# slp-rl/aero

Hardware: AMD Instinct MI355X
Metric: real-time-factor (audio-sec/wall-sec), Aero.forward STFT+U-Net+iSTFT, 4->16kHz nfft=512 hop=64 batch=64 per GPU (higher is better)
Workload: dtype f16; 1 GPU; batch=64 synthetic 2s white-noise clips per GPU, 4->16 kHz, aero_4-16_512_64 (nfft=512 hop=64), random-init weights seed 2036, inference, inputs resident in HBM; global_batch=64, clip_samples=8000, frames=501, parallelism=clips sharded over 1 GPU(s), no data-path collective, precision=fp16 operands/storage, fp32 accumulate; STFT/iSTFT/statistics fp32

## Files before the change

aero_amd/_lib.py:

```python
import ctypes as C
import os

_HERE = os.path.dirname(os.path.abspath(__file__))
DEFAULT_LIB = os.path.join(_HERE, 'libaero_hip.so')

ACT_NONE, ACT_RELU, ACT_GELU, ACT_GLU, ACT_SNAKE = 0, 1, 2, 3, 4

i32, i64, vp, fp, dp = C.c_int32, C.c_int64, C.c_void_p, C.c_void_p, C.c_void_p


class ConvDesc(C.Structure):
    _fields_ = [('src0', vp), ('s0_b', i64), ('s0_f', i64), ('s0_t', i64), ('C0', i32),
                ('src1', vp), ('s1_b', i64), ('s1_f', i64), ('s1_t', i64), ('C1', i32),
                ('weight', vp), ('bias', fp),
                ('dst', vp), ('d_b', i64), ('d_f', i64), ('d_t', i64),
                ('dst_f32', i32), ('dst_f_off', i32), ('dst_F', i32),
                ('B', i32), ('Fin', i32), ('Fout', i32), ('T', i32), ('M', i32),
                ('transposed', i32), ('fstride', i32),
                ('ntaps', i32), ('df', i32 * 9), ('dt', i32 * 9),
                ('act', i32),
                ('res', vp), ('r_b', i64), ('r_f', i64), ('r_t', i64),
                ('post_add', fp), ('batch_scale', fp), ('batch_shift', fp),
                ('stats', dp), ('stat_count', C.c_double),
                ('stat_mode', i32), ('stat_G', i32), ('stat_per_row', i32), ('stat_eps', C.c_float),
# ... 98 lines not shown
    _fields_ = [('xn', vp), ('u', vp), ('g', vp), ('rs', fp), ('a_re', fp), ('a_im', fp), ('bias_f', fp),
                ('wc', vp), ('bias_c', fp), ('dst', vp),
                ('B', i32), ('F', i32), ('T', i32), ('C', i32), ('M', i32), ('Fo', i32), ('ktaps', i32), ('stride', i32),
                ('pad', i32), ('act', i32)]


class SeanetConvDesc(C.Structure):
    _fields_ = [('x', vp), ('wimg', vp), ('bias', fp), ('add', vp), ('y', vp),
                ('B', i32), ('Tin', i32), ('Cin', i32), ('Tq', i32), ('M', i32), ('K', i32), ('stride', i32), ('dil', i32), ('pad', i32),
                ('reflect', i32), ('ksteps', i32), ('R', i32), ('P', i32), ('Tout', i32), ('Cout', i32), ('act', i32), ('in_slope', C.c_float)]


class SeanetResDesc(C.Structure):
    _fields_ = [('x', vp), ('w1', vp), ('w2s', vp), ('b1', fp), ('b2s', fp), ('add', vp), ('y', vp),
                ('B', i32), ('T', i32), ('C', i32), ('d', i32), ('ks1', i32), ('ks2', i32), ('slope', C.c_float)]


DCONV_MAX_DEPTH = 4


class DconvLayer(C.Structure):
    _fields_ = [('w1', vp), ('w2', vp), ('consts', fp), ('snake_a', fp),
                ('dilation', i32), ('norm1', i32), ('norm2', i32), ('reserved', i32)]


class DconvDesc(C.Structure):
    _fields_ = [('x', vp), ('y', vp), ('R', i32), ('T', i32), ('C', i32), ('hidden', i32), ('depth', i32), ('act', i32),
                ('F', i32), ('eps', C.c_float), ('layer', DconvLayer * DCONV_MAX_DEPTH)]


class DconvRewriteDesc(C.Structure):
    _fields_ = [('dconv', DconvDesc), ('rw_w', vp), ('rw_bias', fp), ('post_add', fp),
                ('dst', vp), ('d_b', i64), ('d_f', i64), ('d_t', i64)]


_PROTOS = {
    'aero_version': (C.c_char_p, []),
    'aero_last_error': (C.c_char_p, []),
    'aero_last_kernel_name': (C.c_char_p, []),
    'aero_stft_fwd': (i32, [fp, i32, i32, i32, i32, i32, fp, i32, fp, i32, dp, i32, vp]),
    'aero_stft_dft_table_bytes': (i64, [i32]),
    'aero_stft_dft_table': (i32, [fp, i32, i32, vp, vp]),
    'aero_stft_dft_fwd': (i32, [fp, i32, i32, i32, i32, i32, i32, vp, fp, i32, dp, i32, vp]),
    'aero_stft_dft_norm_fwd': (i32, [fp, i32, i32, i32, i32, i32, i32, vp, i32, dp, i32, vp, fp, vp]),
    'aero_spec_normalize': (i32, [fp, i32, i64, dp, vp, fp, vp]),
    'aero_istft_fwd': (i32, [fp, i32, i32, i32, i32, i32, fp, fp, fp, i32, vp]),
    'aero_istft_pitch': (i32, [i32, i32, i32, C.POINTER(i32), C.POINTER(i32)]),
    'aero_istft_pitched_fwd': (i32, [fp, i32, i32, i32, i32, i32, i32, i32, fp, fp, fp, i32, vp]),
    'aero_conv_fwd': (i32, [C.POINTER(ConvDesc), vp]),
    'aero_split_finish': (i32, [fp, i32, fp, i32, vp, i64, i32, vp]),
    'aero_adam_step': (i32, [fp, fp, fp, fp, i64, C.c_float, C.c_float, C.c_float, C.c_float, i32, C.c_float, vp]),
    'aero_adam_step_dev': (i32, [fp, fp, fp, fp, i64, C.c_float, C.c_float, C.c_float, C.c_float, fp, C.c_float, vp]),
    'aero_conv_wgrad': (i32, [C.POINTER(WgradDesc), vp]),
    'aero_conv_wgrad_chunks': (i32, [i32, i32, i32, i32, i32]),
    'aero_norm_bwd_reduce': (i32, [C.POINTER(NormBwdDesc), vp]),
    'aero_norm_bwd_apply': (i32, [C.POINTER(NormBwdDesc), vp]),
    'aero_istft_bwd_prep': (i32, [fp, fp, fp, i32, i32, i32, i32, i32, vp]),
    'aero_istft_bwd_pack': (i32, [fp, fp, i32, i32, i32, i32, i32, vp]),
    'aero_conv_tile_m': (i32, [i32]),
    'aero_conv_ring_bm': (i32, [i32, i32]),
    'aero_convtr_tail_finish': (i32, [fp, fp, fp, fp, fp, fp, i32, i32, i32, i32, i32, vp]),
    'aero_convtr_tail_finish_pitched': (i32, [fp, fp, fp, fp, fp, fp, i32, i32, i32, i32, i32, i32, i32, vp]),
    'aero_conv_kernel_name': (i32, [C.POINTER(ConvDesc), C.c_char_p, i32]),
    'aero_norm_stats': (i32, [C.POINTER(NormDesc), vp]),
    'aero_norm_apply': (i32, [C.POINTER(NormDesc), vp]),
    'aero_gram_stats': (i32, [C.POINTER(GramDesc), vp]),
    'aero_lstm_fwd': (i32, [C.POINTER(LstmDesc), vp]),
    'aero_lstm_geometry': (i32, [i32, C.POINTER(i32), C.POINTER(i32)]),
    'aero_lstm_geometry_in': (i32, [i32, i32, C.POINTER(i32)]),
    'aero_localstate_fwd': (i32, [C.POINTER(AttnDesc), vp]),
    'aero_freqfc_fwd': (i32, [C.POINTER(FreqFcDesc), vp]),
    'aero_ftb_first_fwd': (i32, [C.POINTER(FtbFirstDesc), vp]),
    'aero_enc0_fwd': (i32, [C.POINTER(Enc0Desc), vp]),
    'aero_dconv_row_fwd': (i32, [C.POINTER(DconvDesc), vp]),
    'aero_dconv_row_fits': (i32, [i32, i32, i32, i32]),
    'aero_dconv_row_rewrite_fwd': (i32, [C.POINTER(DconvRewriteDesc), vp]),
    'aero_dconv_row_rewrite_fits': (i32, [i32, i32, i32, i32]),
    'aero_lstm_bwd': (i32, [C.POINTER(LstmBwdDesc), vp]),
    'aero_lstm_bwd_k4p': (i32, [i32]),
    'aero_localstate_bwd': (i32, [C.POINTER(AttnBwdDesc), vp]),
    'aero_freqfc_wgrad': (i32, [vp, vp, vp, fp, fp, i32, i32, i32, i32, i32, vp]),
    'aero_ftb_gate_bwd': (i32, [vp, vp, vp, vp, vp, vp, i32, i32, i32, i32, vp]),
    'aero_sum_bt': (i32, [vp, fp, i32, i32, i32, i32, C.c_float, vp]),
    'aero_frames_op': (i32, [vp, vp, i32, i32, i32, i32, i32, i32, i32, vp]),
    'aero_stft_loss_sums': (i32, [fp, fp, i64, C.c_float, dp, i32, dp, vp]),
    'aero_stft_loss_bwd': (i32, [fp, fp, i64, C.c_float, dp, C.c_float, C.c_float, fp, fp, vp]),
    'aero_irfft_frames': (i32, [fp, i32, i32, i32, i32, fp, fp, vp]),
    'aero_stft_adj_fold': (i32, [fp, fp, i32, i32, i32, i32, i32, i32, vp]),
    'aero_add_f16': (i32, [vp, vp, vp, i64, C.c_float, vp]),
    'aero_scale_cast': (i32, [fp, i32, i64, fp, vp, C.c_float, vp, fp, vp]),
    'aero_scale_f32': (i32, [fp, i64, fp, vp]),
    'aero_gather_pack': (i32, [vp, vp, i32, vp, vp, i64, i32, vp]),
    'aero_debug_probe': (i32, [vp, i32, i32, i32, vp, vp]),
    'aero_bn_running_update': (i32, [dp, i32, C.c_double, C.c_float, fp, fp, vp, vp]),
    'aero_gconv1d_mfma_ok': (i32, [i32, i32, i32, i32, i32, i32, i32]),
    'aero_weightnorm_fwd': (i32, [fp, fp, fp, i32, i32, vp]),
    'aero_weightnorm_bwd': (i32, [fp, i64, i64, i64, fp, fp, fp, fp, fp, fp, fp, fp, i32, i32, i32, i32, vp]),
    'aero_gconv1d_wgrad_slabs': (i32, [i32, i32, i32, i32, i32, i32, i32, i32, i32]),
    'aero_rescale_f16': (i32, [vp, fp, vp, fp, i64, vp, C.c_float, vp, fp, vp]),
    'aero_gconv1d_fwd': (i32, [C.POINTER(GconvDesc), vp]),
    'aero_pw_fwd': (i32, [C.POINTER(PwDesc), vp]),
    'aero_comm_unique_id': (i32, [vp]),
    'aero_comm_init': (i32, [i32, i32, vp, C.POINTER(vp)]),
    'aero_allreduce_f32': (i32, [vp, fp, i64, vp]),
    'aero_allgather': (i32, [vp, vp, vp, i64, vp]),
    'aero_comm_destroy': (i32, [vp]),
    'aero_stream_create': (i32, [i32, C.POINTER(C.c_uint32), i32, C.POINTER(vp)]),
    'aero_stream_destroy': (i32, [vp]),
    'aero_pw_rows': (i32, [i32, i32]),
    'aero_pw_ksteps': (i32, [i32]),
# ... 78 lines not shown
```

aero_amd/csrc/aero_hip.hip:

```cpp
#include "aero_common.h"
#ifdef AERO_PART
#define AERO_IN(p) (AERO_PART == (p))
#else
#define AERO_IN(p) 1
#endif
#if AERO_IN(0)
#include "k_attn.h"
#include "k_lstm.h"
#include "k_norm.h"
#include "k_gram.h"
#include "k_optim.h"
#endif
#if AERO_IN(1)
#include "k_stft.h"
#include "k_train.h"
#endif
#if AERO_IN(2)
#include "k_conv.h"
#endif
#if AERO_IN(6)
#include "k_conv_ring.h"
#endif
#if AERO_IN(7)
#include "k_pw.h"
// ... 414 lines not shown
int aero_split_finish(const float* acc, int32_t nsplit, const float* bias, int32_t act, void* dst, int64_t npos, int32_t M, void* stream) {
    const char* err = "";
    int rc = aero_split_finish_launch(acc, nsplit, bias, act, dst, npos, M, (hipStream_t)stream, &err);
    return aero_finish(rc, err);
}

#endif

#if AERO_IN(3)

int aero_freqfc_fwd(const aero_freqfc_desc* d, void* stream) {
    const char* err = "";
    int rc = aero_freqfc_launch(d, (hipStream_t)stream, &err);
    return aero_finish(rc, err);
}

int aero_dconv_row_fwd(const aero_dconv_desc* d, void* stream) {
    const char* err = "";
    int rc = aero_dconv_launch(d, nullptr, (hipStream_t)stream, &err);
    return aero_finish(rc, err);
}

int aero_dconv_row_fits(int T, int C, int hidden, int max_dilation) { return aero_dconv_row_fits_impl(T, C, hidden, max_dilation); }

int aero_dconv_row_rewrite_fwd(const aero_dconv_rewrite_desc* d, void* stream) {
    const char* err = "";
    if (!d) return aero_fail(AERO_ERR_ARG, "dconv rewrite: null descriptor");
    int rc = aero_dconv_launch(&d->dconv, d, (hipStream_t)stream, &err);
    return aero_finish(rc, err);
}

int aero_dconv_row_rewrite_fits(int T, int C, int hidden, int max_dilation) { return aero_dconv_row_fits_impl(T, C, hidden, max_dilation, true); }

int aero_enc0_fwd(const aero_enc0_desc* d, void* stream) {
    const char* err = "";
    int rc = aero_enc0_launch(d, (hipStream_t)stream, &err);
    return aero_finish(rc, err);
}

int aero_ftb_first_fwd(const aero_ftb_first_desc* d, void* stream) {
    const char* err = "";
    int rc = aero_ftb_first_launch(d, (hipStream_t)stream, &err);
    return aero_finish(rc, err);
}

#endif

#if AERO_IN(4)

int aero_conv_wgrad(const aero_wgrad_desc* d, void* stream) {
    const char* err = "";
    int rc = aero_conv_wgrad_launch(d, (hipStream_t)stream, &err);
    return aero_finish(rc, err);
}

int aero_conv_wgrad_chunks(int32_t M, int32_t C, int32_t ntaps, int32_t nrows, int32_t T) {
    if (M < 1 || C < 1 || ntaps < 1 || nrows < 1 || T < 1) return 1;
    bool big;
    int nchunk, SC;
    aero_wgrad_plan(M, C, ntaps, nrows, T, &big, &nchunk, &SC);
    return nchunk;
}

int aero_norm_bwd_reduce(const aero_norm_bwd_desc* d, void* stream) {
    const char* err = "";
    int rc = aero_norm_bwd_launch(d, 0, (hipStream_t)stream, &err);
// ... 338 lines not shown
```

aero_amd/csrc/k_dconv.h:

```cpp
#pragma once
#include "aero_common.h"

struct AeroDconvK {
    aero_dconv_desc d;
    int HP;
    int logp;
    int T16;
    int PADR;
    const void* rw_w;
    const float* rw_b;
    const float* rw_add;
    void* out; int64_t o_b, o_f, o_t;
};

static inline int aero_dconv_logp(int C) {
    int s = (2 * C) & 255, g = 256;
    if (s) g = s & -s;
    int P = 256 / g, l = 0;
    while ((1 << l) < P) ++l;
    return l;
}

static inline size_t aero_dconv_lds_bytes(int T, int C, int hidden, int maxdil) {
    if (T < 1 || C < 8 || C % 8 || hidden < 4 || hidden % 4 || hidden > 32 || maxdil < 1 || maxdil > 64) return 0;
// ... 324 lines not shown
    p.rw_b = rw ? rw->rw_bias : nullptr;
    p.rw_add = rw ? rw->post_add : nullptr;
    p.out = rw ? rw->dst : nullptr;
    p.o_b = rw ? rw->d_b : 0; p.o_f = rw ? rw->d_f : 0; p.o_t = rw ? rw->d_t : 0;
    const size_t lds = rw ? aero_dconv_rw_lds_bytes(d->T, d->C, d->hidden, maxdil) : aero_dconv_lds_bytes(d->T, d->C, d->hidden, maxdil);
    const int nw = aero_dconv_nw(lds, d->T), nf2 = d->C / 8;
    dim3 grid((unsigned)d->R), block((unsigned)nw * 64);
#define AERO_DCONV_GO2(NF2_, RW_)                                                                                      \
    do {                                                                                                               \
        constexpr int MF16 = NF2_ >= 12 ? 2 : 4;      \
        if (nw == 16 && (d->T + 15) / 16 > 16 * MF16) { *err = "dconv: row too long"; return AERO_ERR_UNSUPPORTED; }    \
        if (p.HP == 16 && nw == 8) AERO_LAUNCH_DYN((aero_dconv_row_kernel<1, NF2_, 8, 4, RW_>), grid, block, lds, stream, p);  \
        else if (p.HP == 16) AERO_LAUNCH_DYN((aero_dconv_row_kernel<1, NF2_, 16, MF16, RW_>), grid, block, lds, stream, p);       \
        else if (nw == 8) AERO_LAUNCH_DYN((aero_dconv_row_kernel<2, NF2_, 8, 4, RW_>), grid, block, lds, stream, p);           \
        else AERO_LAUNCH_DYN((aero_dconv_row_kernel<2, NF2_, 16, MF16, RW_>), grid, block, lds, stream, p);                       \
    } while (0)
#define AERO_DCONV_GO(NF2_)                                                                                            \
    do {                                                                                                               \
        if (rw) AERO_DCONV_GO2(NF2_, true);                                                                            \
        else AERO_DCONV_GO2(NF2_, false);                                                                              \
    } while (0)
    switch (nf2) {
        case 2: AERO_DCONV_GO(2); break;
        case 4: AERO_DCONV_GO(4); break;
        case 6: AERO_DCONV_GO(6); break;
        case 8: AERO_DCONV_GO(8); break;
        case 12: AERO_DCONV_GO(12); break;
        default: AERO_DCONV_GO(16); break;
    }
#undef AERO_DCONV_GO
#undef AERO_DCONV_GO2
    return AERO_OK;
}
```

aero_amd/engine.py:

```python
import ctypes as C
import math
import os

import torch

from . import _lib, pack
from ._lib import ACT_GELU, ACT_GLU, ACT_NONE, ACT_RELU, ACT_SNAKE


def _ptr(t):
    return None if t is None else t.data_ptr()


def _strides4(t):
    assert t.dim() == 4 and (t.shape[3] == 1 or t.stride(3) == 1), (t.shape, t.stride())
    return t.stride(0), t.stride(1), t.stride(2)


_SIDE_STREAMS = {}


def side_streams(device, n):
    dev = torch.device(device)
    if dev.type == 'cuda' and dev.index is None:
# ... 285 lines not shown
            ar[0].zero_()
        ar[1] = ar[2] = 0
        self._cur = ar

    _bwd = None

    def zeros32(self, n, device, dtype=torch.float32):
        ar = self._bwd
        if ar is not None and ar[0].device == torch.device(device):
            m = (n + 3) // 4 * 4
            ar[2] += m
            if ar[1] + m <= ar[0].numel():
                out = ar[0][ar[1]:ar[1] + n]
                ar[1] += m
                return out if dtype == torch.float32 else out.view(dtype)
        return torch.zeros(n, dtype=dtype, device=device)

    def new_stats(self, B, F, G, per_row, device):
        n = (B * F if per_row == 1 else (1 if per_row == 2 else B)) * G * 2
        ar = self._cur
        if ar is not None and ar[0].device == torch.device(device):
            ar[2] += n
            if ar[1] + n <= ar[0].numel():
                out = ar[0][ar[1]:ar[1] + n].view(-1, 2)
                ar[1] += n
                return out
        return torch.zeros(n // 2, 2, dtype=torch.float64, device=device)

    @staticmethod
    def can_fuse_stats(M, G):
        return M % 8 == 0 and (G == 1 or (M % G == 0 and (M // G) % 16 == 0))

    def norm_act(self, x, G, per_row, gamma, beta, act, snake_a=None, layer_scale=None, res=None, normalize=True,
                 f_lo=0, f_cnt=None, eps=1e-5, dst=None, stats=None, dst_strides=None, stat_count=None):
        B, F, T, Cc = x.shape
        d = _lib.NormDesc()
        d.src = _ptr(x)
        d.s_b, d.s_f, d.s_t = _strides4(x)
        d.B, d.F, d.T, d.C, d.G, d.per_row, d.eps = B, F, T, Cc, G, int(per_row), eps
        if normalize:
            d.stat_count = float((1 if per_row == 1 else (B * F if per_row == 2 else F)) * T * (Cc // G))
            if stat_count is not None:
                d.stat_count = float(stat_count)
            if stats is None:
                stats = self.new_stats(B, F, G, per_row, x.device)
                d.stats = _ptr(stats)
                self._call('aero_norm_stats', 'aero_norm_stats_kernel', 0, x.numel() * 2, C.byref(d), self.stream(x))
            d.stats = _ptr(stats)
        f_cnt = F if f_cnt is None else f_cnt
        assert not (per_row and (f_lo or f_cnt != F))
        Cout = Cc // 2 if act == ACT_GLU else Cc
        out = dst if dst is not None else torch.empty(B, f_cnt, T, Cout, dtype=torch.float16, device=x.device)
        assert dst_strides is not None or out.shape == (B, f_cnt, T, Cout)
        d.src = x.data_ptr() + f_lo * x.stride(1) * x.element_size()
        d.F = f_cnt
        d.gamma, d.beta = _ptr(gamma), _ptr(beta)
        d.act = act
        d.snake_a, d.layer_scale = _ptr(snake_a), _ptr(layer_scale)
        d.res = _ptr(res)
        if res is not None:
            d.r_b, d.r_f, d.r_t = _strides4(res)
        d.dst = _ptr(out)
        d.d_b, d.d_f, d.d_t = dst_strides if dst_strides is not None else _strides4(out)
        self._last_stats = stats
        self._call('aero_norm_apply', 'aero_norm_apply_kernel', 0,
                   B * f_cnt * T * (Cc + Cout + (Cout if res is not None else 0)) * 2, C.byref(d), self.stream(x))
        return out
# ... 85 lines not shown

Ops.enc0 = _enc0


def _dconv_row(self, x, layers, act, F, eps=1e-5, rewrite=None, post_add=None):
    B, Fq, T, Cc = x.shape
    out = torch.empty_like(x)
    r = _lib.DconvRewriteDesc()
    d = r.dconv
    d.x, d.y = _ptr(x), (None if rewrite is not None else _ptr(out))
    d.R, d.T, d.C, d.hidden, d.depth, d.act, d.F, d.eps = B * Fq, T, Cc, layers[0]['hidden'], len(layers), act, F, eps
    flops = 0.0
    for i, L in enumerate(layers):
        l = d.layer[i]
        l.w1, l.w2, l.consts, l.snake_a = _ptr(L['w1']), _ptr(L['w2']), _ptr(L['consts']), _ptr(L.get('snake_a'))
        l.dilation, l.norm1, l.norm2 = L['dilation'], L['norm1'], L['norm2']
        flops += 2.0 * B * Fq * T * L['hidden'] * (3 * Cc + 2 * Cc)
    if rewrite is None:
        self._shape_note = f'dconv rows C={Cc} hidden={layers[0]["hidden"]} depth={len(layers)} F={Fq}'
        self._call('aero_dconv_row_fwd', 'aero_dconv_row_kernel', flops, 2 * x.numel() * 2, C.byref(d), self.stream(x))
        return out
    r.rw_w, r.rw_bias, r.post_add, r.dst = _ptr(rewrite['w']), _ptr(rewrite['bias']), _ptr(post_add), _ptr(out)
    r.d_b, r.d_f, r.d_t = _strides4(out)
    self._shape_note = f'dconv rows + rewrite C={Cc} hidden={layers[0]["hidden"]} depth={len(layers)} F={Fq}'
    self._call('aero_dconv_row_rewrite_fwd', 'aero_dconv_row_kernel', flops + 2.0 * B * Fq * T * 2 * Cc * Cc, 2 * x.numel() * 2, C.byref(r), self.stream(x))
    return out


def _dconv_row_fits(self, T, Cc, hidden, maxdil, rewrite=False):
    fn = self.lib.cdll.aero_dconv_row_rewrite_fits if rewrite else self.lib.cdll.aero_dconv_row_fits
    return bool(fn(T, Cc, hidden, maxdil))


Ops.dconv_row = _dconv_row
Ops.dconv_row_fits = _dconv_row_fits


def blstm_frames(T, W=200, S=100):
    n = math.ceil(T / S)
    if n >= 3 and T <= (n - 1) * S + S // 2:
        n -= 1
    return n


def _hann_padded(win_length, n_fft, device):
    w = torch.zeros(n_fft, dtype=torch.float32)
    left = (n_fft - win_length) // 2
    w[left:left + win_length] = torch.hann_window(win_length, periodic=True, dtype=torch.float32)
    return w.to(device)


class _ShapeCache(dict):
    BOUNDED = ('hidpad', 'ones', 'env', 'graph')
    MAX_PER_KIND = 8

    def __getitem__(self, key):
        v = dict.__getitem__(self, key)
        if isinstance(key, tuple) and key and key[0] in self.BOUNDED:
            dict.__delitem__(self, key)
            dict.__setitem__(self, key, v)
        return v

    def __setitem__(self, key, value):
        dict.__setitem__(self, key, value)
        if isinstance(key, tuple) and key and key[0] in self.BOUNDED:
            same = [k for k in self if isinstance(k, tuple) and k and k[0] == key[0]]
            for k in same[:max(0, len(same) - self.MAX_PER_KIND)]:
                dict.__delitem__(self, k)


class HipEngine:
    use_pw = os.environ.get('AERO_PW', '1') != '0'
    stagger = 0
    prof_streams = False
    stage_hook = None
    lstm_frame_major = os.environ.get('AERO_LSTM_FRAME_MAJOR', '1') != '0'
    _mark_base = None
    _out_pitch = None

    def __init__(self, model, lib=None):
        self.model = model
        self.lib = lib if lib is not None else _lib.load()
        self.ops = Ops(self.lib)
        self._key = None
        self._params, self._epoch = None, 0
        self._tables = _ShapeCache()
        self.streams = int(os.environ.get('AERO_STREAMS', '0'))
        self.stagger = int(os.environ.get('AERO_STAGGER', '0'))
        self.prof_streams = False
        self.use_graph = os.environ.get('AERO_GRAPH', '0') != '0'
        self.fuse_dconv_tail = os.environ.get('AERO_FUSE_DCONV', '1') != '0'
        self.gram_stats = os.environ.get('AERO_GRAM_STATS', '1') != '0'
        self.fuse_stats = {'0': False, '1': True}.get(os.environ.get('AERO_FUSE_STATS', 'auto'), 'auto')
        self.ring_stats = os.environ.get('AERO_RING_STATS', '1') != '0'
        self.fuse_lstm_proj = True
        self.collapse_first_ftb = True
        self.split_taps = os.environ.get('AERO_TAP_SPLIT', '1') != '0'
        self.use_pw = os.environ.get('AERO_PW', '1') != '0'
        self.fuse_dconv_row = os.environ.get('AERO_DCONV_ROW', '1') != '0'
        self.fuse_dconv_rewrite = os.environ.get('AERO_DCONV_ROW_REWRITE', '1') != '0'
        self.fuse_enc0 = os.environ.get('AERO_FUSE_ENC0', '1') != '0'
        self.fuse_tail = os.environ.get('AERO_FUSE_TAIL', '1') != '0'
        self.pitched_out = os.environ.get('AERO_PITCHED_OUT', '1') != '0'

    def _weights_key(self, device):
        if self._params is None:
            self._params = list(self.model.state_dict(keep_vars=True).values())
        return (str(device), self._epoch) + tuple((p.data_ptr(), p._version) for p in self._params)

    def invalidate(self):
        self._epoch += 1
        self._params = None

    def _prepare(self, device):
        key = self._weights_key(device)
        if key != self._key:
            self._params = None
            self._pack(device)
            self._key = key
            for k in [k for k in self._tables if isinstance(k, tuple) and k and k[0] == 'graph']:
                del self._tables[k]

    def _pack(self, device):
        m = self.model
        sd = {k: v.detach().float().cpu() for k, v in m.state_dict().items()}
        P = {}
        mk = pack.make_conv_spec
        for i, enc in enumerate(m.encoder):
            p = f'encoder.{i}'
            L = {}
            if enc.is_first:
                w, df, dt = pack.conv2d_taps(sd[f'{p}.pre_conv.weight'], 0, 0)
                L['pre'] = mk(w, sd[f'{p}.pre_conv.bias'], w.shape[-1], 0, df, dt, device)
# ... 80 lines not shown
                              fstride=dec.stride, act=act)
            if dec.last and not dec.norm and dec.rewrite is not None:
                timg = pack.convtr_tail_image(sd[f'{p}.conv_tr.weight'], dec.stride, device)
                rw = L['rewrite']
                if (timg is not None and rw.M == 192 and rw.tiled_bm == 192 and len(rw.df) == 9 and timg.shape[1] == 96 and dec.pad == 2
                        and dec.kernel_size == 8):
                    L['tail'] = (timg, sd[f'{p}.conv_tr.bias'].detach().float().to(device).contiguous())
            if not dec.last and os.environ.get('AERO_CONVTR_STACK', '1') != '0':
                st = pack.convtr_stacked_spec(sd[f'{p}.conv_tr.weight'], sd[f'{p}.conv_tr.bias'], dec.stride, device, act=act)
                if st is not None:
                    L['conv_tr_stacked'] = st
            if dec.norm:
                L['norm2'] = (sd[f'{p}.norm2.weight'].to(device), sd[f'{p}.norm2.bias'].to(device))
            if dec.dconv is not None:
                raise NotImplementedError('decoder DConv (dconv_mode & 2) is not used by any reference config')
            P[p] = L
        if m.freq_emb is not None:
            emb = sd['freq_emb.embedding.weight'] * m.freq_emb.scale * m.freq_emb_scale
            P['freq_emb'] = emb.to(device).contiguous()
        self.P = P

    def _pack_dconv(self, sd, p, dc, device):
        mk = pack.make_conv_spec
        out = []
        for d in range(dc.depth):
            q = f'{p}.layers.{d}'
            dil = 2 ** d if dc.dilate else 1
            L = {}
            w, df, dt = pack.conv1d_taps(sd[f'{q}.conv1.0.weight'], dil, dil * (dc.kernel // 2))
            L['conv1'] = mk(w, sd[f'{q}.conv1.0.bias'], w.shape[-1], 0, df, dt, device)
            L['gn1'] = (sd[f'{q}.conv1.1.weight'].to(device), sd[f'{q}.conv1.1.bias'].to(device)) if dc.norm else None
            if dc.act_func == 'snake':
                L['snake_a'] = sd[f'{q}.act.a'].reshape(-1).to(device).contiguous()
            if dc.lstm:
                H = dc.hidden
                L['lstm'] = [pack.pack_lstm_layer(self.lib, sd, f'{q}.lstm.lstm', l, H, device) for l in range(2)]
                w = sd[f'{q}.lstm.linear.weight']
                L['lstm_lin'] = mk(w[None, :, None, :], sd[f'{q}.lstm.linear.bias'], w.shape[1], 0, [0], [0], device)
                L['lstm_lin_pw'] = pack.make_pw_spec(w, sd[f'{q}.lstm.linear.bias'], ACT_NONE, self.lib, device)
            if dc.time_attn:
                a = f'{q}.time_attn'
                w = torch.cat([sd[f'{a}.{n}.weight'][:, :, 0] for n in ('query', 'key', 'content', 'query_decay')], 0)
                b = torch.cat([sd[f'{a}.{n}.bias'] for n in ('query', 'key', 'content', 'query_decay')], 0)
                L['attn_qkvd'] = mk(w[None, :, None, :], b, w.shape[1], 0, [0], [0], device)
                L['attn_qkvd_pw'] = pack.make_pw_spec(w, b, ACT_NONE, self.lib, device)
                w = sd[f'{a}.proj.weight'][:, :, 0]
                L['attn_proj'] = mk(w[None, :, None, :], sd[f'{a}.proj.bias'], w.shape[1], 0, [0], [0], device)
                L['attn_proj_pw'] = pack.make_pw_spec(w, sd[f'{a}.proj.bias'], ACT_NONE, self.lib, device)
                mod = dc.layers[d]['time_attn']
                L['attn_geom'] = (mod.heads, mod.ndecay)
            w, df, dt = pack.conv1d_taps(sd[f'{q}.conv2.0.weight'], 1, 0)
            L['conv2'] = mk(w, sd[f'{q}.conv2.0.bias'], w.shape[-1], 0, df, dt, device)
            L['gn2'] = (sd[f'{q}.conv2.1.weight'].to(device), sd[f'{q}.conv2.1.bias'].to(device)) if dc.norm else None
            L['scale'] = sd[f'{q}.conv2.3.scale'].to(device).contiguous()
            w, df, dt = pack.conv1d_taps(sd[f'{q}.conv2.0.weight'], 1, 0)
            L['conv2_glu'] = mk(w, sd[f'{q}.conv2.0.bias'], w.shape[-1], 0, df, dt, device, act=ACT_GLU)
            L['pw2'] = pack.make_pw_spec(w[0, :, 0, :], sd[f'{q}.conv2.0.bias'], ACT_GLU, self.lib, device) if (dc.lstm or dc.time_attn) and dc.norm else None
            if dc.norm:
                L['gn2_glu'] = (pack.glu_interleave(sd[f'{q}.conv2.1.weight']).to(device).contiguous(),
                                pack.glu_interleave(sd[f'{q}.conv2.1.bias']).to(device).contiguous())
            hid = w.shape[-1]
            if not dc.lstm and not dc.time_attn and dc.kernel == 3 and hid % 4 == 0 and hid <= 32 and w.shape[1] % 16 == 0:
                g = (lambda n: sd[n]) if dc.norm else (lambda n: None)
                L['row'] = pack.dconv_row_layer(sd[f'{q}.conv1.0.weight'], sd[f'{q}.conv1.0.bias'], g(f'{q}.conv1.1.weight'),
                                                g(f'{q}.conv1.1.bias'), sd[f'{q}.conv2.0.weight'][:, :, 0], sd[f'{q}.conv2.0.bias'],
                                                g(f'{q}.conv2.1.weight'), g(f'{q}.conv2.1.bias'), sd[f'{q}.conv2.3.scale'], dil, device)
# ... 79 lines not shown
                st.wait_event(prev_events[self.stagger])
            events = {}

            def stage_cb(i, events=events, st=st):
                if i == self.stagger:
                    ev = torch.cuda.Event()
                    ev.record(st)
                    events[i] = ev
            with torch.cuda.stream(st):
                outs.append(self._forward_one(part, want_spec, want_lr_spec, defer_istft=True, stage_cb=stage_cb if self.stagger else None))
            prev_events = events
        for st in self._tables[key]:
            cur.wait_stream(st)
        ys = []
        for o in outs:
            spec_out, hop, win, T, Lout = o[0]
            spec_out.record_stream(cur)
            y = self.ops.istft(spec_out, self.model.nfft, hop, self._window(win, mix.device), self._inv_env(win, hop, T, mix.device), Lout)
            ys.append(y.view(spec_out.shape[0], 1, Lout))
        res = [torch.cat(ys, 0)]
        for k in (1, 2):
            parts = [o[k] for o in outs]
            if parts[0] is None:
                res.append(None)
                continue
            for t in parts:
                t.record_stream(cur)
            res.append(torch.cat(parts, 0))
        return tuple(res)

    def _forward_graph(self, mix, want_spec, want_lr_spec):
        key = ('graph', tuple(mix.shape), str(mix.device), want_spec, want_lr_spec,
               self.fuse_dconv_tail, self.fuse_stats, self.collapse_first_ftb, self.fuse_lstm_proj, self.fuse_enc0, self.fuse_dconv_row, self.fuse_dconv_rewrite,
               self.split_taps)
        self._prepare(mix.device)
        ent = self._tables.get(key)
        if ent is None:
            static_in = mix.clone()
            for _ in range(2):
                self._forward_one(static_in, want_spec, want_lr_spec)
            torch.cuda.synchronize(mix.device)
            g = torch.cuda.CUDAGraph()
            with torch.cuda.graph(g):
                static_out = self._forward_one(static_in, want_spec, want_lr_spec)
            ent = self._tables[key] = (g, static_in, static_out)
        g, static_in, static_out = ent
        static_in.copy_(mix)
        g.replay()
        return tuple(None if t is None else t.clone() for t in static_out)

    def _forward_one(self, mix, want_spec=False, want_lr_spec=False, train=False, defer_istft=False, stage_cb=None):
        m, ops, P = self.model, self.ops, None
        self._train = train
        if stage_cb is None:
            stage_cb = self.stage_hook
        self._check_input(mix)
        if m.in_channels != 1 or m.out_channels != 1:
            raise NotImplementedError('only in_channels = out_channels = 1 (all reference configs)')
        dev = mix.device
        self._prepare(dev)
        P = self.P
        B, _, L = mix.shape
        mix = mix.contiguous()
        ops.begin_step(dev)
        stats = ops.new_stats(B, 1, 1, False, dev)
        fused = None
        if not want_lr_spec:
# ... 193 lines not shown
                else:
                    y = ops.conv(L['rewrite'], y, None, B, Fo, Fo, T, post_add=emb)
                ops.tag = ''
        elif i == 0 and 'freq_emb' in self.P:
            raise NotImplementedError('frequency embedding without a rewrite conv')
        return y, Fo

    def _row_rewrite_applies(self, enc, L, y, T):
        layers = L['dconv']
        if not (getattr(self, 'fuse_dconv_rewrite', False) and self.fuse_dconv_row and self.use_pw and not enc.norm
                and not getattr(self, '_train', False) and L.get('rewrite_row') is not None and y.is_contiguous()
                and all('row' in Lr for Lr in layers) and len(layers) <= _lib.DCONV_MAX_DEPTH):
            return False
        r0 = layers[0]['row']
        if L['rewrite_row']['C'] != r0['C']:
            return False
        maxdil = max(Lr['row']['dilation'] for Lr in layers)
        return self.ops.dconv_row_fits(T, r0['C'], r0['hidden'], maxdil) and self.ops.dconv_row_fits(T, r0['C'], r0['hidden'], maxdil, rewrite=True)

    def _mark(self, stage):
        if self.stage_hook is not None and not getattr(self, '_train', False):
            self.stage_hook(stage)

    def _dconv(self, dc, layers, x, B, Fo, T):
        ops = self.ops
        act = {'snake': ACT_SNAKE, 'gelu': ACT_GELU}.get(dc.act_func, ACT_RELU)
        if (self.fuse_dconv_row and all('row' in L for L in layers) and len(layers) <= _lib.DCONV_MAX_DEPTH and x.is_contiguous()
                and ops.dconv_row_fits(T, layers[0]['row']['C'], layers[0]['row']['hidden'], max(L['row']['dilation'] for L in layers))):
            return ops.dconv_row(x, [dict(L['row'], snake_a=L.get('snake_a')) for L in layers], act, Fo)
        for li, L in enumerate(layers):
            if li == 1 and getattr(self, '_mark_base', None) is not None:
                self._mark(self._mark_base + 0.5)
            g1 = L['gn1']
            st1 = None
            if g1 is not None and self._want_stats(L['conv1']) and L['conv1'].M > 16 and L['conv1'].M % 8 == 0:
                st1 = ops.new_stats(B, Fo, 1, True, x.device)
                h = ops.conv(L['conv1'], x, None, B, Fo, Fo, T, stat=dict(mode=1, stats=st1, G=1, per_row=True))
            else:
                h = ops.conv(L['conv1'], x, None, B, Fo, Fo, T)
            g2 = L['gn2']
            hp = L.get('hid_pad') if (g2 is not None and self.fuse_dconv_tail and L['conv2_glu'].M % 16 == 0) else None
            hdst = None
            if hp:
                hid = h.shape[-1]
                key = ('hidpad', B, Fo, T, hp, str(x.device), self.ops.stream(x))
                if key not in self._tables:
                    self._tables[key] = torch.zeros(B, Fo, T, hp, dtype=torch.float16, device=x.device)
                hdst = self._tables[key][..., :hid]
            h = ops.norm_act(h, 1, True, g1[0] if g1 else None, g1[1] if g1 else None, act,
                             snake_a=L.get('snake_a'), normalize=g1 is not None, stats=st1, dst=hdst)
            if hp:
                st2 = ops.new_stats(B, Fo, 1, True, x.device)
                c2, hb = L['conv2_glu_pad'], self._tables[key]
                if self.gram_stats and 'gram_pad' in L:
                    ops.gram_stats(hb, L['gram_pad'], st2)
                else:
                    ops.conv(c2, hb, None, B, Fo, Fo, T, act=ACT_NONE, stat=dict(mode=2, stats=st2, G=1, per_row=True))
                x = ops.conv(c2, hb, None, B, Fo, Fo, T, res=x,
                             stat=dict(mode=3, stats=st2, G=1, per_row=True, count=float(T * c2.M),
                                       gamma=L['gn2_glu'][0], beta=L['gn2_glu'][1], layer_scale=L['scale']))
                continue
            if 'lstm' in L:
                h = self._blstm(dc, L, h, B, Fo, T)
            if 'attn_qkvd' in L:
                heads, ndecay = L['attn_geom']
                pwq, pwp = (L.get('attn_qkvd_pw'), L.get('attn_proj_pw')) if (self.use_pw and h.is_contiguous()) else (None, None)
                qkvd = ops.pw(pwq, h, B, Fo, T) if pwq is not None else ops.conv(L['attn_qkvd'], h, None, B, Fo, Fo, T)
                att = ops.localstate(qkvd, B * Fo, T, dc.hidden, heads, ndecay)
                if pwp is not None:
                    h = ops.pw(pwp, att.view(B, Fo, T, dc.hidden), B, Fo, T, res=h)
                else:
                    h = ops.conv(L['attn_proj'], att.view(B, Fo, T, dc.hidden), None, B, Fo, Fo, T, res=h)
            if g2 is not None and self.fuse_dconv_tail and L['conv2_glu'].M % 16 == 0 and L['conv2_glu'].C0 % 8 == 0:
                st2 = ops.new_stats(B, Fo, 1, True, x.device)
                c2 = L['conv2_glu']
                if self.gram_stats and 'gram' in L:
                    ops.gram_stats(h, L['gram'], st2)
                else:
                    ops.conv(c2, h, None, B, Fo, Fo, T, act=ACT_NONE, stat=dict(mode=2, stats=st2, G=1, per_row=True))
                if self.use_pw and L.get('pw2') is not None and h.is_contiguous():
                    x = ops.pw(L['pw2'], h, B, Fo, T, res=x, stats=st2, count=float(T * c2.M), gamma=L['gn2_glu'][0],
                               beta=L['gn2_glu'][1], layer_scale=L['scale'])
                    continue
# ... 117 lines not shown
```

aero_amd/pack.py:

```python
import math
from dataclasses import dataclass, field
from typing import List, Optional

import torch

from . import _lib


@dataclass
class ConvSpec:
    weight: torch.Tensor
    bias: Optional[torch.Tensor]
    M: int
    C0: int
    C1: int
    df: List[int]
    dt: List[int]
    transposed: int = 0
    fstride: int = 1
    act: int = _lib.ACT_NONE
    extra: dict = field(default_factory=dict)
    weight_tiled: Optional[torch.Tensor] = None
    tiled_bm: int = 0

# ... 205 lines not shown
    if KPI is not None:
        wih = torch.zeros(2, MP, KPI, device=w_ih.device)
        for dr in range(2):
            wih[dr, :4 * H, :in_ch] = w_ih[dr * 4 * H:(dr + 1) * 4 * H]
        fused = (wih.to(device=device, dtype=torch.float16).contiguous(), b.float().to(device).contiguous(), in_ch)
    return spec, b.to(device=device, dtype=torch.float16).contiguous(), \
        whh.to(device=device, dtype=torch.float16).contiguous(), fused


def dconv_row_layer(w1, b1, g1, be1, w2, b2, g2, be2, scale, dilation, device):
    hid, Cc = w1.shape[0], w1.shape[1]
    HP, K1p = _round_up(hid, 16), _round_up(3 * Cc, 32)
    i1 = torch.zeros(HP, K1p)
    i1[:hid, :3 * Cc] = w1.detach().float().permute(0, 2, 1).reshape(hid, 3 * Cc)
    i2 = torch.zeros(2 * Cc, HP)
    i2[:, :hid] = glu_interleave(w2.detach().float())
    i2 = i2.reshape(2 * Cc // 16, 16, HP // 16, 4, 4).permute(0, 2, 3, 1, 4).contiguous()
    c = torch.zeros(3 * HP + 7 * Cc)
    c[:hid] = b1.detach().float()
    c[HP:HP + hid] = 1.0 if g1 is None else g1.detach().float()
    if be1 is not None:
        c[2 * HP:2 * HP + hid] = be1.detach().float()
    o = 3 * HP
    c[o:o + 2 * Cc] = glu_interleave(b2.detach().float())
    c[o + 2 * Cc:o + 4 * Cc] = 1.0 if g2 is None else glu_interleave(g2.detach().float())
    if be2 is not None:
        c[o + 4 * Cc:o + 6 * Cc] = glu_interleave(be2.detach().float())
    c[o + 6 * Cc:] = 1.0 if scale is None else scale.detach().float()
    return dict(w1=i1.to(device=device, dtype=torch.float16).contiguous(), w2=i2.to(device=device, dtype=torch.float16).contiguous(),
                consts=c.to(device).contiguous(), norm1=int(g1 is not None), norm2=int(g2 is not None), dilation=int(dilation),
                C=Cc, hidden=hid)


def dconv_rewrite_image(w, bias, device):
    M, Cc = w.shape
    if M != 2 * Cc or Cc % 16:
        return None
    ks = (Cc + 31) // 32
    wi = torch.zeros(M, ks * 32)
    wi[:, :Cc] = glu_interleave(w.detach().float().cpu())
    img = wi.reshape(M // 16, 16, ks, 4, 8).permute(0, 2, 3, 1, 4).contiguous()
    b = torch.zeros(M) if bias is None else glu_interleave(bias.detach().float().cpu())
    return dict(w=img.to(device=device, dtype=torch.float16).contiguous(), bias=b.to(device).contiguous(), C=Cc)
```

include/aero_hip.h:

```cpp
#ifndef AERO_HIP_H
#define AERO_HIP_H
#include <stdint.h>

#ifdef __cplusplus
extern "C" {
#endif

#define AERO_OK 0
#define AERO_ERR_ARG (-1)
#define AERO_ERR_LAUNCH (-2)
#define AERO_ERR_UNSUPPORTED (-3)

enum { AERO_ACT_NONE = 0, AERO_ACT_RELU = 1, AERO_ACT_GELU = 2, AERO_ACT_GLU = 3, AERO_ACT_SNAKE = 4 };

const char* aero_version(void);
const char* aero_last_error(void);
const char* aero_last_kernel_name(void);

int aero_stft_fwd(const float* x, int32_t nsig, int32_t L, int32_t Lp, int32_t n_fft, int32_t hop,
                  const float* window, int32_t n_bins, float* spec, int32_t T, double* stats,
                  int32_t sig_per_item, void* stream);

int64_t aero_stft_dft_table_bytes(int32_t n_fft);
int aero_stft_dft_table(const float* window, int32_t n_fft, int32_t win_off, void* table, void* stream);
// ... 118 lines not shown
int aero_ftb_first_fwd(const aero_ftb_first_desc* d, void* stream);

typedef struct {
    const void* xn; const void* u; const void* g;
    const float* rs; const float* a_re; const float* a_im; const float* bias_f;
    const void* wc; const float* bias_c;
    void* dst;
    int32_t B, F, T, C, M, Fo, ktaps, stride, pad, act;
} aero_enc0_desc;
int aero_enc0_fwd(const aero_enc0_desc* d, void* stream);

#define AERO_DCONV_MAX_DEPTH 4
typedef struct {
    const void* w1; const void* w2; const float* consts; const float* snake_a;
    int32_t dilation, norm1, norm2, reserved;
} aero_dconv_layer;
typedef struct {
    const void* x; void* y;
    int32_t R, T, C, hidden, depth, act, F;
    float eps;
    aero_dconv_layer layer[AERO_DCONV_MAX_DEPTH];
} aero_dconv_desc;
int aero_dconv_row_fwd(const aero_dconv_desc* d, void* stream);
int aero_dconv_row_fits(int T, int C, int hidden, int max_dilation);

typedef struct {
    aero_dconv_desc dconv;
    const void* rw_w; const float* rw_bias; const float* post_add;
    void* dst; int64_t d_b, d_f, d_t;
} aero_dconv_rewrite_desc;
int aero_dconv_row_rewrite_fwd(const aero_dconv_rewrite_desc* d, void* stream);
int aero_dconv_row_rewrite_fits(int T, int C, int hidden, int max_dilation);

int aero_adam_step(float* p, const float* g, float* m, float* v, int64_t n, float lr, float beta1, float beta2, float eps,
                   int32_t step, float grad_scale, void* stream);
int aero_adam_step_dev(float* p, const float* g, float* m, float* v, int64_t n, float lr, float beta1, float beta2, float eps,
                       const float* bc, float grad_scale, void* stream);


typedef struct {
    const void* dy; int64_t dy_b, dy_f, dy_t;
    const void* x; int64_t x_b, x_f, x_t;
    float* dw; float* db;
    int32_t B, Fin, Fout, T, M, C, ntaps, fstride;
    int32_t df[9], dt[9];
    float* slabs; int32_t nslab;
    int32_t store, dw_layout, dw_rowlen, dw_coff;
} aero_wgrad_desc;
int aero_conv_wgrad(const aero_wgrad_desc* d, void* stream);
int aero_conv_wgrad_chunks(int32_t M, int32_t C, int32_t ntaps, int32_t nrows, int32_t T);

typedef struct {
    const void* x; int64_t x_b, x_f, x_t;
    const void* dy; int64_t dy_b, dy_f, dy_t;
    void* dx; int64_t dx_b, dx_f, dx_t;
    int32_t B, F, T, C, G, per_row;
    float eps;
    const double* stats; double stat_count;
    const float* gamma; const float* beta; const float* layer_scale;
    int32_t act;
    double* sums;
    float* dgamma; float* dbeta; float* dlayer_scale;
    const float* snake_a; float* dsnake_a;
    double* psums;
} aero_norm_bwd_desc;
int aero_norm_bwd_reduce(const aero_norm_bwd_desc* d, void* stream);
// ... 137 lines not shown
```

Baseline: 15370 audio-sec/wall-sec.

## Fuse dconv first conv, per-row GroupNorm and activation into one kernel

Adds a new HIP kernel that runs the dilated 3-tap conv1 of each dconv layer with MFMA, computes the per-row group-norm statistics in registers, then applies gamma/beta and the activation before writing fp16 output. It replaces a conv kernel with stats, followed by a separate norm/act kernel, and removes the intermediate hidden-tensor round trip through HBM and one launch. Each block handles one (b,f) row with 16 waves and a 3-stage LDS ring fed by async global-to-LDS loads. The cost is a one-block-per-row grid and large LDS use, which may reduce occupancy. The path applies only at inference within shape limits (T<=512, hidden<=96).

```diff
diff --git a/aero_amd/_lib.py b/aero_amd/_lib.py
--- a/aero_amd/_lib.py
+++ b/aero_amd/_lib.py
@@ -154,6 +154,14 @@
 class DconvRewriteDesc(C.Structure):
     _fields_ = [('dconv', DconvDesc), ('rw_w', vp), ('rw_bias', fp), ('post_add', fp),
                 ('dst', vp), ('d_b', i64), ('d_f', i64), ('d_t', i64)]
+
+
+class DconvHeadDesc(C.Structure):
+    _fields_ = [('x', vp), ('s_b', i64), ('s_f', i64), ('s_t', i64),
+                ('w', vp), ('bias', fp), ('gamma', fp), ('beta', fp), ('snake_a', fp),
+                ('dst', vp), ('d_b', i64), ('d_f', i64), ('d_t', i64),
+                ('B', i32), ('F', i32), ('T', i32), ('C', i32), ('hidden', i32), ('dilation', i32), ('act', i32),
+                ('eps', C.c_float)]
 
 
 _PROTOS = {
@@ -198,6 +206,8 @@
     'aero_dconv_row_fits': (i32, [i32, i32, i32, i32]),
     'aero_dconv_row_rewrite_fwd': (i32, [C.POINTER(DconvRewriteDesc), vp]),
     'aero_dconv_row_rewrite_fits': (i32, [i32, i32, i32, i32]),
+    'aero_dconv_head_fwd': (i32, [C.POINTER(DconvHeadDesc), vp]),
+    'aero_dconv_head_fits': (i32, [i32, i32, i32, i32]),
     'aero_lstm_bwd': (i32, [C.POINTER(LstmBwdDesc), vp]),
     'aero_lstm_bwd_k4p': (i32, [i32]),
     'aero_localstate_bwd': (i32, [C.POINTER(AttnBwdDesc), vp]),
diff --git a/aero_amd/csrc/aero_hip.hip b/aero_amd/csrc/aero_hip.hip
--- a/aero_amd/csrc/aero_hip.hip
+++ b/aero_amd/csrc/aero_hip.hip
@@ -470,6 +470,14 @@
 
 int aero_dconv_row_rewrite_fits(int T, int C, int hidden, int max_dilation) { return aero_dconv_row_fits_impl(T, C, hidden, max_dilation, true); }
 
+int aero_dconv_head_fwd(const aero_dconv_head_desc* d, void* stream) {
+    const char* err = "";
+    int rc = aero_dconv_head_launch(d, (hipStream_t)stream, &err);
+    return aero_finish(rc, err);
+}
+
+int aero_dconv_head_fits(int T, int C, int hidden, int dilation) { return aero_dconv_head_lds_bytes(T, C, hidden, dilation) != 0; }
+
 int aero_enc0_fwd(const aero_enc0_desc* d, void* stream) {
     const char* err = "";
     int rc = aero_enc0_launch(d, (hipStream_t)stream, &err);
diff --git a/aero_amd/csrc/k_dconv.h b/aero_amd/csrc/k_dconv.h
--- a/aero_amd/csrc/k_dconv.h
+++ b/aero_amd/csrc/k_dconv.h
@@ -380,3 +380,186 @@
 #undef AERO_DCONV_GO2
     return AERO_OK;
 }
+
+struct AeroDconvHeadK {
+    aero_dconv_head_desc d;
+    int T16, xrows;
+    int stage;
+};
+
+#define AERO_DCONV_HEAD_NW 16
+#define AERO_DCONV_HEAD_STAGES 3
+
+static inline size_t aero_dconv_head_lds_bytes(int T, int C, int hidden, int dilation) {
+    if (T < 1 || T > 16 * AERO_DCONV_HEAD_NW * 2 || C < 32 || C % 32 || hidden < 16 || hidden % 16 || hidden > 96 || dilation < 1 || dilation > 8) return 0;
+    const int T16 = (T + 15) / 16 * 16;
+    const size_t stage = (size_t)(T16 + 16) * 32 + (size_t)3 * (hidden / 16) * 512;
+    return AERO_DCONV_HEAD_STAGES * stage * 2 + AERO_DCONV_HEAD_NW * 2 * sizeof(float);
+}
+
+static __device__ __forceinline__ void aero_dconv_head_wait(int n) {
+    if (n == 1) aero_wait_vm<1>();
+    else if (n == 2) aero_wait_vm<2>();
+    else if (n == 3) aero_wait_vm<3>();
+    else if (n == 4) aero_wait_vm<4>();
+    else aero_wait_vm<0>();
+}
+
+template <int HM>
+__global__ __launch_bounds__(AERO_DCONV_HEAD_NW * 64) void aero_dconv_head_kernel(AeroDconvHeadK p) {
+    constexpr int NW = AERO_DCONV_HEAD_NW, NT = NW * 64, NS = AERO_DCONV_HEAD_STAGES, MAXF = 2, PADR = 8, hidden = HM * 16;
+    const aero_dconv_head_desc& d = p.d;
+    const int T = d.T, C = d.C, dil = d.dilation;
+    h16* ring = (h16*)AERO_DYN_SMEM;
+    float* red = (float*)(ring + NS * p.stage);
+    const int tid = threadIdx.x, lane = tid & 63, wave = aero_uniform(tid >> 6);
+    const int g = lane >> 4, col = lane & 15;
+    const int row = (int)blockIdx.x, b = row / d.F, f = row - b * d.F;
+    const int nfrag = p.T16 >> 4, NK = C >> 5;
+    const int ngx = p.xrows >> 4, ng = ngx + 3 * HM;
+    const int nmine = wave < ng ? (ng - wave + NW - 1) / NW : 0;
+    const h16* src = (const h16*)d.x + (int64_t)b * d.s_b + (int64_t)f * d.s_f;
+
+    auto issue = [&](int kk) {
+        h16* st = ring + (kk % NS) * p.stage;
+        for (int grp = wave; grp < ng; grp += NW) {
+            const h16* sp;
+            if (grp < ngx) {
+                const int U = grp * 64 + lane, r = U >> 2, q = (U & 3) ^ ((0 - (r >> 2)) & 3), t = r - PADR;
+                sp = (t >= 0 && t < T) ? src + (int64_t)t * d.s_t + kk * 32 + q * 8 : aero_zero_page;
+            } else {
+                sp = (const h16*)d.w + ((int64_t)kk * 3 * HM * 64 + (grp - ngx) * 64 + lane) * 8;
+            }
+            aero_glds16(sp, st + grp * 512);
+        }
+    };
+
+    f32x4 acc[MAXF][HM];
+    {
+        f32x4 seed[HM];
+#pragma unroll
+        for (int mf = 0; mf < HM; ++mf) seed[mf] = *(const f32x4*)&d.bias[mf * 16 + g * 4];
+#pragma unroll
+        for (int fi = 0; fi < MAXF; ++fi)
+#pragma unroll
+            for (int mf = 0; mf < HM; ++mf) acc[fi][mf] = seed[mf];
+    }
+    float snake_a = 0.f, snake_ia = 0.f;
+    if (d.act == AERO_ACT_SNAKE) { snake_a = d.snake_a[f]; snake_ia = 1.0f / snake_a; }
+    aero_pin(snake_a, snake_ia);
+#ifndef AERO_EMU
+#pragma unroll
+    for (int mf = 0; mf < HM; ++mf) asm volatile("" : "+v"(acc[0][mf]), "+v"(acc[1][mf]));
+#endif
+
+    issue(0);
+    if (NK > 1) issue(1);
+    int rbase[MAXF];
+#pragma unroll
+    for (int fi = 0; fi < MAXF; ++fi) { const int cf = wave + fi * NW; rbase[fi] = (cf < nfrag ? cf : nfrag - 1) * 16 + col + PADR; }
+    for (int kk = 0; kk < NK; ++kk) {
+        aero_dconv_head_wait(kk + 1 < NK ? nmine : 0);
+        aero_phase_barrier();
+        if (kk + 2 < NK) issue(kk + 2);
+        const h16* xs = ring + (kk % NS) * p.stage;
+        const h16* ws = xs + p.xrows * 32 + lane * 8;
+        h16x8 a[2][HM], bf[2][MAXF];
+        auto fetch = [&](int tap, int s) {
+#pragma unroll
+            for (int mf = 0; mf < HM; ++mf) a[s][mf] = *(const h16x8*)&ws[(tap * HM + mf) * 512];
+#pragma unroll
+            for (int fi = 0; fi < MAXF; ++fi) bf[s][fi] = *(const h16x8*)&xs[aero_tile_off(rbase[fi] + (tap - 1) * dil, g)];
+        };
+        fetch(0, 0);
+#pragma unroll
+        for (int tap = 0; tap < 3; ++tap) {
+            if (tap + 1 < 3) fetch(tap + 1, (tap + 1) & 1);
+#pragma unroll
+            for (int fi = 0; fi < MAXF; ++fi)
+#pragma unroll
+                for (int mf = 0; mf < HM; ++mf) acc[fi][mf] = __builtin_amdgcn_mfma_f32_16x16x32_f16(a[tap & 1][mf], bf[tap & 1][fi], acc[fi][mf], 0, 0, 0);
+        }
+    }
+
+    float s1 = 0.f, s2 = 0.f;
+#pragma unroll
+    for (int fi = 0; fi < MAXF; ++fi) {
+        const int cf = wave + fi * NW;
+        const float msk = (cf < nfrag && cf * 16 + col < T) ? 1.f : 0.f;
+#pragma unroll
+        for (int mf = 0; mf < HM; ++mf) {
+            const f32x4 hv = acc[fi][mf];
+            s1 = fmaf(msk, (hv[0] + hv[1]) + (hv[2] + hv[3]), s1);
+            s2 = fmaf(msk, fmaf(hv[0], hv[0], hv[1] * hv[1]) + fmaf(hv[2], hv[2], hv[3] * hv[3]), s2);
+        }
+    }
+    s1 = aero_wave_sum(s1);
+    s2 = aero_wave_sum(s2);
+    if (lane == 0) { red[wave * 2] = s1; red[wave * 2 + 1] = s2; }
+    __syncthreads();
+    float mean, rstd;
+    {
+        float sa = 0.f, sb = 0.f;
+#pragma unroll
+        for (int w = 0; w < NW; ++w) { sa += red[w * 2]; sb += red[w * 2 + 1]; }
+        aero_dconv_moments(sa, sb, 1.0f / ((float)hidden * (float)T), d.eps, mean, rstd);
+    }
+    h16* img = ring;
+#pragma unroll
+    for (int mf = 0; mf < HM; ++mf) {
+        const f32x4 ga = *(const f32x4*)&d.gamma[mf * 16 + g * 4] * rstd;
+        const f32x4 gb = *(const f32x4*)&d.beta[mf * 16 + g * 4] - ga * mean;
+#pragma unroll
+        for (int fi = 0; fi < MAXF; ++fi) {
+            const int cf = wave + fi * NW;
+            if (cf >= nfrag) continue;
+            h16x4 o;
+#pragma unroll
+            for (int e = 0; e < 4; ++e) {
+                float y = fmaf(acc[fi][mf][e], ga[e], gb[e]);
+                if (d.act == AERO_ACT_GELU) y = aero_gelu(y);
+                else if (d.act == AERO_ACT_RELU) y = fmaxf(y, 0.f);
+                else if (d.act == AERO_ACT_SNAKE) { const float sn = aero_fast_sin(y * snake_a); y = y + (sn * sn) * snake_ia; }
+                o[e] = (h16)y;
+            }
+            *(h16x4*)&img[(cf * 16 + col) * hidden + mf * 16 + g * 4] = o;
+        }
+    }
+    __syncthreads();
+    {
+        constexpr int HV = hidden / 8;
+        h16* dst = (h16*)d.dst + (int64_t)b * d.d_b + (int64_t)f * d.d_f;
+        for (int u = tid; u < T * HV; u += NT) {
+            const int t = u / HV, s = u - t * HV;
+            *(h16x8*)(dst + (int64_t)t * d.d_t + s * 8) = *(const h16x8*)&img[t * hidden + s * 8];
+        }
+    }
+}
+
+static int aero_dconv_head_launch(const aero_dconv_head_desc* d, hipStream_t stream, const char** err) {
+    if (!d || !d->x || !d->w || !d->bias || !d->gamma || !d->beta || !d->dst) { *err = "dconv head: null pointer"; return AERO_ERR_ARG; }
+    if (d->B < 1 || d->F < 1 || d->T < 1) { *err = "dconv head: bad geometry"; return AERO_ERR_ARG; }
+    if (d->act != AERO_ACT_RELU && d->act != AERO_ACT_GELU && d->act != AERO_ACT_SNAKE && d->act != AERO_ACT_NONE) { *err = "dconv head: unsupported act"; return AERO_ERR_UNSUPPORTED; }
+    if (d->act == AERO_ACT_SNAKE && !d->snake_a) { *err = "dconv head: snake needs a"; return AERO_ERR_ARG; }
+    const size_t lds = aero_dconv_head_lds_bytes(d->T, d->C, d->hidden, d->dilation);
+    if (!lds) { *err = "dconv head: C % 32, hidden % 16, hidden > 96, dilation > 8 or T > 512"; return AERO_ERR_UNSUPPORTED; }
+    if ((((uintptr_t)d->x | (uintptr_t)d->w | (uintptr_t)d->bias | (uintptr_t)d->gamma | (uintptr_t)d->beta | (uintptr_t)d->dst) & 15) ||
+        ((d->s_b | d->s_f | d->s_t | d->d_b | d->d_f | d->d_t) & 7) || d->s_t < d->C || d->d_t < d->hidden)
+        { *err = "dconv head: unaligned pointers / strides"; return AERO_ERR_ARG; }
+    if ((int64_t)d->B * d->F > 0x7fffffff) { *err = "dconv head: grid too large"; return AERO_ERR_ARG; }
+    AeroDconvHeadK p;
+    p.d = *d;
+    p.T16 = (d->T + 15) / 16 * 16;
+    p.xrows = p.T16 + 16;
+    p.stage = p.xrows * 32 + 3 * (d->hidden / 16) * 512;
+    dim3 grid((unsigned)(d->B * d->F)), block(AERO_DCONV_HEAD_NW * 64);
+    switch (d->hidden / 16) {
+        case 1: AERO_LAUNCH_DYN((aero_dconv_head_kernel<1>), grid, block, lds, stream, p); break;
+        case 2: AERO_LAUNCH_DYN((aero_dconv_head_kernel<2>), grid, block, lds, stream, p); break;
+        case 3: AERO_LAUNCH_DYN((aero_dconv_head_kernel<3>), grid, block, lds, stream, p); break;
+        case 4: AERO_LAUNCH_DYN((aero_dconv_head_kernel<4>), grid, block, lds, stream, p); break;
+        case 5: AERO_LAUNCH_DYN((aero_dconv_head_kernel<5>), grid, block, lds, stream, p); break;
+        default: AERO_LAUNCH_DYN((aero_dconv_head_kernel<6>), grid, block, lds, stream, p); break;
+    }
+    return AERO_OK;
+}
diff --git a/aero_amd/engine.py b/aero_amd/engine.py
--- a/aero_amd/engine.py
+++ b/aero_amd/engine.py
@@ -341,7 +341,10 @@
         return M % 8 == 0 and (G == 1 or (M % G == 0 and (M // G) % 16 == 0))
 
     def norm_act(self, x, G, per_row, gamma, beta, act, snake_a=None, layer_scale=None, res=None, normalize=True,
-                 f_lo=0, f_cnt=None, eps=1e-5, dst=None, stats=None, dst_strides=None, stat_count=None):
+                 f_lo=0, f_cnt=None, eps=1e-5, dst=None, stats=None, dst_strides=None, stat_count=None, head=None):
+        if head is not None:
+            assert G == 1 and per_row == 1 and normalize and stats is None and res is None and layer_scale is None and not f_lo and f_cnt is None
+            return self.dconv_head(x, head[0], act, snake_a=snake_a, eps=eps, dst=dst, dilation=head[1])
         B, F, T, Cc = x.shape
         d = _lib.NormDesc()
         d.src = _ptr(x)
@@ -493,8 +496,30 @@
     return bool(fn(T, Cc, hidden, maxdil))
 
 
+def _dconv_head(self, x, H, act, snake_a=None, eps=1e-5, dst=None, dilation=None):
+    B, Fq, T, Cc = x.shape
+    hid, dil = H['hidden'], (H['dilation'] if dilation is None else int(dilation))
+    out = dst if dst is not None else torch.empty(B, Fq, T, hid, dtype=torch.float16, device=x.device)
+    assert out.shape == (B, Fq, T, hid) and Cc == H['C']
+    d = _lib.DconvHeadDesc()
+    d.x, d.w, d.bias, d.gamma, d.beta, d.snake_a, d.dst = _ptr(x), _ptr(H['w']), _ptr(H['bias']), _ptr(H['gamma']), _ptr(H['beta']), _ptr(snake_a), _ptr(out)
+    d.s_b, d.s_f, d.s_t = _strides4(x)
+    d.d_b, d.d_f, d.d_t = _strides4(out)
+    d.B, d.F, d.T, d.C, d.hidden, d.dilation, d.act, d.eps = B, Fq, T, Cc, hid, dil, act, eps
+    npos = B * Fq * T
+    self._shape_note = f'dconv head C={Cc} hidden={hid} dilation={dil} F={Fq}'
+    self._call('aero_dconv_head_fwd', 'aero_dconv_head_kernel', 2.0 * npos * hid * 3 * Cc, 2 * npos * (Cc + hid), C.byref(d), self.stream(x))
+    return out
+
+
+def _dconv_head_fits(self, T, Cc, hidden, dilation):
+    return bool(self.lib.cdll.aero_dconv_head_fits(T, Cc, hidden, dilation))
+
+
 Ops.dconv_row = _dconv_row
 Ops.dconv_row_fits = _dconv_row_fits
+Ops.dconv_head = _dconv_head
+Ops.dconv_head_fits = _dconv_head_fits
 
 
 def blstm_frames(T, W=200, S=100):
@@ -560,6 +585,7 @@
         self.use_pw = os.environ.get('AERO_PW', '1') != '0'
         self.fuse_dconv_row = os.environ.get('AERO_DCONV_ROW', '1') != '0'
         self.fuse_dconv_rewrite = os.environ.get('AERO_DCONV_ROW_REWRITE', '1') != '0'
+        self.fuse_dconv_head = os.environ.get('AERO_DCONV_HEAD', '1') != '0'
         self.fuse_enc0 = os.environ.get('AERO_FUSE_ENC0', '1') != '0'
         self.fuse_tail = os.environ.get('AERO_FUSE_TAIL', '1') != '0'
         self.pitched_out = os.environ.get('AERO_PITCHED_OUT', '1') != '0'
@@ -706,6 +732,9 @@
             L['gn1'] = (sd[f'{q}.conv1.1.weight'].to(device), sd[f'{q}.conv1.1.bias'].to(device)) if dc.norm else None
             if dc.act_func == 'snake':
                 L['snake_a'] = sd[f'{q}.act.a'].reshape(-1).to(device).contiguous()
+            if dc.norm and dc.kernel == 3:
+                L['head'] = pack.dconv_head_image(sd[f'{q}.conv1.0.weight'], sd[f'{q}.conv1.0.bias'], sd[f'{q}.conv1.1.weight'],
+                                                  sd[f'{q}.conv1.1.bias'], dil, device)
             if dc.lstm:
                 H = dc.hidden
                 L['lstm'] = [pack.pack_lstm_layer(self.lib, sd, f'{q}.lstm.lstm', l, H, device) for l in range(2)]
@@ -851,7 +880,7 @@
     def _forward_graph(self, mix, want_spec, want_lr_spec):
         key = ('graph', tuple(mix.shape), str(mix.device), want_spec, want_lr_spec,
                self.fuse_dconv_tail, self.fuse_stats, self.collapse_first_ftb, self.fuse_lstm_proj, self.fuse_enc0, self.fuse_dconv_row, self.fuse_dconv_rewrite,
-               self.split_taps)
+               self.split_taps, self.fuse_dconv_head, self.pitched_out, self.ops.fused_stft, self.lstm_frame_major)
         self._prepare(mix.device)
         ent = self._tables.get(key)
         if ent is None:
@@ -1111,8 +1140,13 @@
             if li == 1 and getattr(self, '_mark_base', None) is not None:
                 self._mark(self._mark_base + 0.5)
             g1 = L['gn1']
+            H, dil1 = L.get('head'), max(L['conv1'].dt)
+            fused_head = (getattr(self, 'fuse_dconv_head', False) and not getattr(self, '_train', False) and g1 is not None and H is not None
+                          and x.is_contiguous() and list(L['conv1'].dt) == [-dil1, 0, dil1] and ops.dconv_head_fits(T, H['C'], H['hidden'], dil1))
             st1 = None
-            if g1 is not None and self._want_stats(L['conv1']) and L['conv1'].M > 16 and L['conv1'].M % 8 == 0:
+            if fused_head:
+                h = None
+            elif g1 is not None and self._want_stats(L['conv1']) and L['conv1'].M > 16 and L['conv1'].M % 8 == 0:
                 st1 = ops.new_stats(B, Fo, 1, True, x.device)
                 h = ops.conv(L['conv1'], x, None, B, Fo, Fo, T, stat=dict(mode=1, stats=st1, G=1, per_row=True))
             else:
@@ -1121,13 +1155,16 @@
             hp = L.get('hid_pad') if (g2 is not None and self.fuse_dconv_tail and L['conv2_glu'].M % 16 == 0) else None
             hdst = None
             if hp:
-                hid = h.shape[-1]
+                hid = L['conv1'].M
                 key = ('hidpad', B, Fo, T, hp, str(x.device), self.ops.stream(x))
                 if key not in self._tables:
                     self._tables[key] = torch.zeros(B, Fo, T, hp, dtype=torch.float16, device=x.device)
                 hdst = self._tables[key][..., :hid]
-            h = ops.norm_act(h, 1, True, g1[0] if g1 else None, g1[1] if g1 else None, act,
-                             snake_a=L.get('snake_a'), normalize=g1 is not None, stats=st1, dst=hdst)
+            if fused_head:
+                h = ops.norm_act(x, 1, True, g1[0], g1[1], act, snake_a=L.get('snake_a'), dst=hdst, head=(H, dil1))
+            else:
+                h = ops.norm_act(h, 1, True, g1[0] if g1 else None, g1[1] if g1 else None, act,
+                                 snake_a=L.get('snake_a'), normalize=g1 is not None, stats=st1, dst=hdst)
             if hp:
                 st2 = ops.new_stats(B, Fo, 1, True, x.device)
                 c2, hb = L['conv2_glu_pad'], self._tables[key]
diff --git a/aero_amd/pack.py b/aero_amd/pack.py
--- a/aero_amd/pack.py
+++ b/aero_amd/pack.py
@@ -261,6 +261,16 @@
                 C=Cc, hidden=hid)
 
 
+def dconv_head_image(w1, b1, g1, be1, dilation, device):
+    hid, Cc, k = w1.shape
+    if k != 3 or Cc % 32 or hid % 16 or hid > 96 or g1 is None or not 1 <= dilation <= 8:
+        return None
+    img = w1.detach().float().cpu().reshape(hid // 16, 16, Cc // 32, 4, 8, 3).permute(2, 5, 0, 3, 1, 4).contiguous()
+    f = lambda v: v.detach().float().to(device).contiguous()
+    return dict(w=img.to(device=device, dtype=torch.float16).contiguous(), bias=f(b1), gamma=f(g1), beta=f(be1), dilation=int(dilation),
+                C=Cc, hidden=hid)
+
+
 def dconv_rewrite_image(w, bias, device):
     M, Cc = w.shape
     if M != 2 * Cc or Cc % 16:
diff --git a/include/aero_hip.h b/include/aero_hip.h
--- a/include/aero_hip.h
+++ b/include/aero_hip.h
@@ -174,6 +174,16 @@
 int aero_dconv_row_rewrite_fwd(const aero_dconv_rewrite_desc* d, void* stream);
 int aero_dconv_row_rewrite_fits(int T, int C, int hidden, int max_dilation);
 
+typedef struct {
+    const void* x; int64_t s_b, s_f, s_t;
+    const void* w; const float* bias; const float* gamma; const float* beta; const float* snake_a;
+    void* dst; int64_t d_b, d_f, d_t;
+    int32_t B, F, T, C, hidden, dilation, act;
+    float eps;
+} aero_dconv_head_desc;
+int aero_dconv_head_fwd(const aero_dconv_head_desc* d, void* stream);
+int aero_dconv_head_fits(int T, int C, int hidden, int dilation);
+
 int aero_adam_step(float* p, const float* g, float* m, float* v, int64_t n, float lr, float beta1, float beta2, float eps,
                    int32_t step, float grad_scale, void* stream);
 int aero_adam_step_dev(float* p, const float* g, float* m, float* v, int64_t n, float lr, float beta1, float beta2, float eps,
```

Measured after the change: 15410 audio-sec/wall-sec, median of 6. Within noise of the previous version (+0.2%).
